# chanchanchan97/ICAFusion

Measured on AMD Instinct MI355X. Metric: RGB/IR image-pairs/sec (two-stream forward + NMS), higher is better.
Workload: dtype bf16

## Files before the change

icafusion_amd/_lib.py:

```python
import ctypes as C
import os

_HERE = os.path.dirname(os.path.abspath(__file__))
LIB_PATH = os.environ.get("ICAF_LIB") or os.path.join(_HERE, "lib", "libicaf.so")

F32, BF16, F16 = 0, 1, 2
ACT_NONE, ACT_SILU, ACT_GELU = 0, 1, 2


class ConvArgs(C.Structure):
    _fields_ = [
        ("x", C.c_void_p), ("w", C.c_void_p), ("bias", C.c_void_p), ("y", C.c_void_p), ("res", C.c_void_p),
        ("x_gs", C.c_longlong), ("w_gs", C.c_longlong), ("bias_gs", C.c_longlong), ("y_gs", C.c_longlong),
        ("res_gs", C.c_longlong),
        ("groups", C.c_int),
        ("B", C.c_int), ("H", C.c_int), ("W", C.c_int), ("Cin", C.c_int), ("ldx", C.c_int),
        ("Ho", C.c_int), ("Wo", C.c_int), ("Cout", C.c_int), ("ldy", C.c_int),
        ("kh", C.c_int), ("kw", C.c_int), ("sh", C.c_int), ("sw", C.c_int), ("ph", C.c_int), ("pw", C.c_int),
        ("ldr", C.c_int), ("Kp", C.c_int), ("act", C.c_int), ("dtype", C.c_int), ("out_dtype", C.c_int),
        ("alpha_acc", C.c_float * 2), ("alpha_res", C.c_float * 2),
        ("tile", C.c_int),
        ("pre", C.c_void_p), ("pre_h", C.c_int), ("pre_w", C.c_int), ("ldpre", C.c_int), ("pre_mode", C.c_int),
        ("w2", C.c_void_p), ("bias2", C.c_void_p), ("y2", C.c_void_p),
        ("w2_gs", C.c_longlong), ("bias2_gs", C.c_longlong), ("y2_gs", C.c_longlong),
# ... 5 lines not shown

class BneckArgs(C.Structure):
    _fields_ = [("conv", ConvArgs), ("w1", C.c_void_p), ("bias1", C.c_void_p), ("w1_gs", C.c_longlong),
                ("bias1_gs", C.c_longlong), ("Kp1", C.c_int), ("shape", C.c_int),
                ("x2", C.c_void_p), ("x2_gs", C.c_longlong), ("ldx2", C.c_int), ("reserved", C.c_int)]


class Stem2Args(C.Structure):
    _fields_ = [("img", C.c_void_p), ("img_u8", C.c_int), ("ctot", C.c_int),
                ("dtype", C.c_int), ("nstreams", C.c_int), ("B", C.c_int), ("H", C.c_int), ("W", C.c_int),
                ("w0", C.c_void_p), ("bias0", C.c_void_p), ("w0_gs", C.c_longlong), ("bias0_gs", C.c_longlong),
                ("Kp0", C.c_int), ("C0", C.c_int),
                ("w1", C.c_void_p), ("bias1", C.c_void_p), ("w1_gs", C.c_longlong), ("bias1_gs", C.c_longlong),
                ("Kp1", C.c_int), ("C1", C.c_int),
                ("w2", C.c_void_p), ("bias2", C.c_void_p), ("w2_gs", C.c_longlong), ("bias2_gs", C.c_longlong),
                ("Kp2", C.c_int), ("C2", C.c_int),
                ("y", C.c_void_p), ("y_gs", C.c_longlong), ("ldy", C.c_int), ("reserved", C.c_int)]


class DmffArgs(C.Structure):
    _fields_ = [("x", C.c_void_p), ("qkv", C.c_void_p), ("y", C.c_void_p),
                ("wqkv", C.c_void_p), ("bqkv", C.c_void_p), ("wo", C.c_void_p), ("bo", C.c_void_p),
                ("w1", C.c_void_p), ("b1", C.c_void_p), ("w2", C.c_void_p), ("b2", C.c_void_p),
                ("ln_attn_gamma", C.c_void_p * 2), ("ln_attn_beta", C.c_void_p * 2),
                ("ln_mlp_gamma", C.c_void_p), ("ln_mlp_beta", C.c_void_p),
                ("wqkv_gs", C.c_longlong), ("bqkv_gs", C.c_longlong), ("wo_gs", C.c_longlong), ("bo_gs", C.c_longlong),
                ("w1_gs", C.c_longlong), ("b1_gs", C.c_longlong), ("w2_gs", C.c_longlong), ("b2_gs", C.c_longlong),
                ("x_gs", C.c_longlong), ("y_gs", C.c_longlong),
                ("dtype", C.c_int), ("B", C.c_int), ("N", C.c_int), ("C", C.c_int), ("heads", C.c_int), ("Kp", C.c_int),
                ("Kp4", C.c_int), ("hidden", C.c_int), ("ldy", C.c_int), ("reserved", C.c_int),
                ("eps_attn", C.c_float), ("eps_mlp", C.c_float),
                ("coef_res_attn", C.c_float * 2), ("coef_acc_attn", C.c_float * 2),
                ("coef_res_mlp", C.c_float * 2), ("coef_acc_mlp", C.c_float * 2), ("debug_clock", C.c_void_p),
                ("x32", C.c_void_p), ("y32", C.c_void_p)]


class TtaPass(C.Structure):
    _fields_ = [("dst", C.c_void_p), ("Hr", C.c_int), ("Wr", C.c_int), ("Hp", C.c_int), ("Wp", C.c_int), ("flip", C.c_int), ("reserved", C.c_int)]


class FrameGeom(C.Structure):
    _fields_ = [("offset", C.c_longlong), ("h0", C.c_int), ("w0", C.c_int), ("pitch", C.c_int), ("ch", C.c_int), ("nh", C.c_int), ("nw", C.c_int),
                ("top", C.c_int), ("left", C.c_int), ("sx", C.c_float), ("sy", C.c_float)]


LETTERBOX_LDS_BYTES = 20480


_p, _i, _ll, _f, _sz = C.c_void_p, C.c_int, C.c_longlong, C.c_float, C.c_size_t
SIGNATURES = {
    "icaf_last_error": (C.c_char_p, []),
    "icaf_set_option": (_i, [C.c_char_p, _i]),
    "icaf_version": (_i, []),
    "icaf_device_info": (_i, [C.POINTER(_i), C.POINTER(_i), C.c_char_p, _i]),
    "icaf_preprocess_nchw": (_i, [_p, _p, _i, _i, _i, _i, _i, _i, _i, _p]),
    "icaf_preprocess_u8": (_i, [_p, _p, _i, _i, _i, _i, _i, _i, _i, _i, _i, _i, _p]),
    "icaf_stem": (_i, [_p, _i, _i, _p, _p, _p, _i, _i, _i, _i, _i, _i, _i, _i, _ll, _ll, _ll, _p]),
    "icaf_stem2": (_i, [C.POINTER(Stem2Args), _p]),
    "icaf_conv2d": (_i, [C.POINTER(ConvArgs), _p]),
    "icaf_bottleneck": (_i, [C.POINTER(BneckArgs), _p]),
    "icaf_conv2d_kernel_name": (_i, [C.POINTER(ConvArgs), C.c_char_p, _i]),
    "icaf_conv2d_config_ids": (_i, [C.POINTER(_i), _i]),
    "icaf_sppf_pool": (_i, [_p, _i, _p, _p, _p, _i, _i, _i, _i, _i, _i, _i, _p]),
    "icaf_sppf_config": (_i, [_i, _i, _i, _i, C.POINTER(_i)]),
    "icaf_upsample_nearest": (_i, [_p, _i, _p, _i, _i, _i, _i, _i, _i, _i, _p]),
    "icaf_copy_channels": (_i, [_p, _i, _p, _i, _i, _ll, _i, _p]),
    "icaf_axpby": (_i, [_p, _i, _p, _i, _p, _i, _i, _ll, _i, _f, _f, _p]),
    "icaf_dmff_pool_tokens": (_i, [_p, _i, _p, _i, _p, _p, _p, _i, _i, _i, _i, _i, _i, _i, _i, _i, _i, _i,
                                   _f, _f, _f, _f, _p]),
    "icaf_layernorm": (_i, [_p, _p, _p, _p, _p, _p, _i, _ll, _i, _i, _f, _p]),
    "icaf_cross_attention": (_i, [_p, _p, _i, _i, _i, _i, _i, _p]),
    "icaf_cross_attention_config": (_i, [_i, _i, _i, _i, _i, C.POINTER(_i), C.POINTER(_i), C.POINTER(_i)]),
    "icaf_dmff_ln_qkv": (_i, [C.POINTER(DmffArgs), _p]),
    "icaf_dmff_attn_mlp": (_i, [C.POINTER(DmffArgs), _p]),
    "icaf_dmff_wide_ln_qkv": (_i, [C.POINTER(DmffArgs), _p]),
    "icaf_dmff_wide_proj_mlp": (_i, [C.POINTER(DmffArgs), _p, _p]),
    "icaf_dmff_wide_proj_mlp_split": (_i, [C.POINTER(DmffArgs), _p, _p, _i, _p]),
    "icaf_dmff_wide_reduce": (_i, [C.POINTER(DmffArgs), _p, _i, _p]),
    "icaf_dmff_attn_mlp_lds_bytes": (_i, [_i, _i, _i, _i, C.POINTER(_sz)]),
    "icaf_dmff_upsample_merge": (_i, [_p, _p, _i, _p, _i, _p, _i, _i, _i, _i, _i, _i, _i, _i, _p]),
    "icaf_detect_decode": (_i, [_p, _i, _p, _p, _p, _i, _i, _i, _i, _i, _ll, _ll, _f, C.POINTER(_f), _p]),
    "icaf_detect_decode_kernel": (_i, [_p, _i, _p, _p, _i, _i, _i, _i, _i, C.POINTER(_i)]),
    "icaf_detect_conv": (_i, [C.POINTER(ConvArgs), _p, _p, _p, _i, _i, _ll, _ll, _f, C.POINTER(_f), _p]),
    "icaf_tta_stage": (_i, [_p, _i, _i, _i, _i, _i, C.POINTER(TtaPass), _i, _p]),
    "icaf_tta_merge": (_i, [C.POINTER(_p), C.POINTER(_ll), C.POINTER(_f), C.POINTER(_i), _i, _p, _i, _i, _f, _p]),
    "icaf_letterbox_frames": (_i, [_p, _p, _i, _i, _p, _i, _i, _i, _i, _p]),
    "icaf_scale_detections": (_i, [_p, _p, _i, _i, _p, _i, _p, _p]),
    "icaf_match_predictions": (_i, [_p, _p, _i, _i, _p, _p, _i, _p, _p, _i, _p, _p, _p]),
    "icaf_nms_workspace_bytes": (_i, [_i, _ll, _i, _i, C.POINTER(_sz)]),
    "icaf_nms": (_i, [_p, _i, _ll, _i, _f, _f, _i, _i, C.POINTER(_i), _i, _i, _i, _f, _p, _p, _p, _p, _sz, _p]),
    "icaf_graph_begin": (_i, [_p]),
    "icaf_graph_end": (_i, [_p, C.POINTER(_p)]),
    "icaf_graph_launch": (_i, [_p, _p]),
    "icaf_graph_destroy": (_i, [_p]),
    "icaf_event_create": (_i, [C.POINTER(_p)]),
    "icaf_event_record": (_i, [_p, _p]),
    "icaf_stream_wait_event": (_i, [_p, _p]),
    "icaf_event_elapsed_ms": (_i, [_p, _p, C.POINTER(_f)]),
    "icaf_event_destroy": (_i, [_p]),
    "icaf_stream_sync": (_i, [_p]),
}

_LIB = None


class IcafError(RuntimeError):
# ... 30 lines not shown
```

icafusion_amd/csrc/api.hip:

```cpp
#include "icaf_common.h"
#include <cstring>

namespace icaf {
std::string& last_error() {
    static thread_local std::string e;
    return e;
}
int fail(int code, const char* fmt, ...) {
    char buf[1024];
    va_list ap;
    va_start(ap, fmt);
    vsnprintf(buf, sizeof(buf), fmt, ap);
    va_end(ap);
    last_error() = buf;
    return code;
}
LibOptions g_opt;
}

using namespace icaf;

extern "C" const char* icaf_last_error(void) { return last_error().c_str(); }

extern "C" int icaf_set_option(const char* name, int value) {
    if (!name) return fail(ICAF_ERR_ARG, "icaf_set_option: null name");
    if (!strcmp(name, "detect_elementwise")) g_opt.detect_elementwise = value;
    else if (!strcmp(name, "attn_qsplit")) g_opt.attn_qsplit = value;
    else if (!strcmp(name, "sppf_vpb")) g_opt.sppf_vpb = value;
    else if (!strcmp(name, "letterbox_direct")) g_opt.letterbox_direct = value;
    else return fail(ICAF_ERR_ARG, "icaf_set_option: unknown option '%s' (detect_elementwise, attn_qsplit, sppf_vpb, letterbox_direct)", name);
    return ICAF_OK;
}
extern "C" int icaf_version(void) { return 100; }

extern "C" int icaf_device_info(int* cu_count, int* lds_bytes, char* arch, int arch_len) {
    int dev = 0;
    ICAF_HIP(hipGetDevice(&dev));
    hipDeviceProp_t prop;
    ICAF_HIP(hipGetDeviceProperties(&prop, dev));
    if (cu_count) *cu_count = prop.multiProcessorCount;
    if (lds_bytes) *lds_bytes = (int)prop.sharedMemPerBlock;
    if (arch && arch_len > 0) {
        strncpy(arch, prop.gcnArchName, arch_len - 1);
        arch[arch_len - 1] = 0;
    }
    return ICAF_OK;
}

extern "C" int icaf_graph_begin(icaf_stream_t s) {
    ICAF_HIP(hipStreamBeginCapture(S(s), hipStreamCaptureModeThreadLocal));
    return ICAF_OK;
}
extern "C" int icaf_graph_end(icaf_stream_t s, void** graph_exec) {
    hipGraph_t graph = nullptr;
    ICAF_HIP(hipStreamEndCapture(S(s), &graph));
    hipGraphExec_t exec = nullptr;
    hipError_t e = hipGraphInstantiate(&exec, graph, nullptr, nullptr, 0);
    hipGraphDestroy(graph);
    if (e != hipSuccess) return fail(ICAF_ERR_HIP, "hipGraphInstantiate -> %s", hipGetErrorString(e));
    *graph_exec = (void*)exec;
    return ICAF_OK;
}
extern "C" int icaf_graph_launch(void* graph_exec, icaf_stream_t s) {
    ICAF_HIP(hipGraphLaunch((hipGraphExec_t)graph_exec, S(s)));
    return ICAF_OK;
}
extern "C" int icaf_graph_destroy(void* graph_exec) {
    if (graph_exec) ICAF_HIP(hipGraphExecDestroy((hipGraphExec_t)graph_exec));
    return ICAF_OK;
}
extern "C" int icaf_event_create(void** ev) {
    hipEvent_t e;
    ICAF_HIP(hipEventCreate(&e));
    *ev = (void*)e;
    return ICAF_OK;
}
extern "C" int icaf_event_record(void* ev, icaf_stream_t s) {
    ICAF_HIP(hipEventRecord((hipEvent_t)ev, S(s)));
    return ICAF_OK;
}
extern "C" int icaf_stream_wait_event(icaf_stream_t s, void* ev) {
    ICAF_HIP(hipStreamWaitEvent(S(s), (hipEvent_t)ev, 0));
    return ICAF_OK;
}
extern "C" int icaf_event_elapsed_ms(void* start, void* stop, float* ms) {
    ICAF_HIP(hipEventSynchronize((hipEvent_t)stop));
// ... 12 lines not shown
```

icafusion_amd/csrc/detect.hip:

```cpp
#pragma clang fp contract(off)
#include "icaf_common.h"
#include "stream_core.h"
#include <cstdlib>

namespace icaf {

struct Anchors { float v[16]; };
int conv_prepare(const icaf_conv_args* a, ConvP& p);

struct DetectDiv { FastDiv no, nx, ny, na; };

template <bool I32>
__global__ __launch_bounds__(256) void detect_decode_kernel(const float* __restrict__ p, int ldp, float* __restrict__ z,
                                                            float* __restrict__ logits, float* __restrict__ raw, int B, int ny, int nx,
                                                            int na, int no, long long rows_total, long long row_offset, float stride,
                                                            Anchors anc, DetectDiv dv) {
    const long long total = (long long)B * na * ny * nx * no;
    for (long long e = (long long)blockIdx.x * blockDim.x + threadIdx.x; e < total; e += (long long)gridDim.x * blockDim.x) {
        int o, x, y, a, b;
        if constexpr (I32) {
            unsigned int q, r;
            fd_divmod((unsigned int)e, dv.no, q, r);
            o = (int)r;
            fd_divmod(q, dv.nx, q, r);
// ... 107 lines not shown
            const int nl = col0 + 8 * qd + 4 * hi;
#pragma unroll
            for (int b = 0; b < TM; ++b) {
                const int ml = row0 + b * 32 + l31;
                f32x4 v;
#pragma unroll
                for (int j = 0; j < 4; ++j) v[j] = acc[b][4 * qd + j] + bq[qd][j];
                *(f32x4*)(stg + ml * SO + nl * 4) = v;
            }
        }
    }
    __device__ __forceinline__ void flush(const unsigned char* stg, int m0, int n0, int tid) const {
        if (tid >= 128 * NA) return;
        const int row = tid / NA, a = tid - row * NA;
        const unsigned int pix = (unsigned int)(m0 + row);
        if ((int)pix >= M) return;
        unsigned int t, x, b, y;
        fd_divmod(pix, dnx, t, x);
        fd_divmod(t, dny, b, y);
        const float* src = (const float*)(stg + row * SO) + a * NO;
        float v[NO];
#pragma unroll
        for (int k = 0; k < NO; k += 2) { const float2 q2 = *(const float2*)(src + k); v[k] = q2.x; v[k + 1] = q2.y; }
        const long long cell = ((long long)a * ny + y) * nx + x;
        const long long zrow = (long long)b * rows_total + row_offset + cell;
        float o[NO];
#pragma unroll
        for (int k = 0; k < NO; ++k) {
            const float sg = 1.0f / (1.0f + expf(-v[k]));
            float out = sg;
            if (k == 0) out = ((sg * 2.0f - 0.5f) + (float)x) * stride;
            else if (k == 1) out = ((sg * 2.0f - 0.5f) + (float)y) * stride;
            else if (k == 2 || k == 3) {
                const float d = sg * 2.0f;
                out = (d * d) * anc.v[2 * a + (k - 2)];
            }
            o[k] = out;
        }
        float* zr = z + zrow * NO;
#pragma unroll
        for (int k = 0; k < NO; k += 2) *(float2*)(zr + k) = float2{o[k], o[k + 1]};
        if (raw) {
            float* rr = raw + (((long long)b * NA) * ny * nx + cell) * NO;
#pragma unroll
            for (int k = 0; k < NO; k += 2) *(float2*)(rr + k) = float2{v[k], v[k + 1]};
        }
        if (logits) {
#pragma unroll
            for (int k = 5; k < NO; ++k) logits[zrow * (NO - 5) + (k - 5)] = v[k];
        }
    }
};

template <int DT, int NA, int NO>
__global__ __launch_bounds__(512) void detect_conv_kernel(const ConvP p, const DetectEpi<NA, NO> epi) {
    stream_gemm<DT, 64, 1>(p, epi);
}

template <int DT, int NA, int NO>
static int launch_detect_conv(const ConvP& p, const DetectEpi<NA, NO>& epi, hipStream_t s) {
    constexpr int LDS = 3 * (128 + 64) * 128 + 128 * DetectEpi<NA, NO>::SO;
    ConvP q = p;
    q.mtiles = (p.M + 127) / 128;
    q.ntiles = 1;
    q.nchunks = p.K / 64;
    int dev = 0, cus = 256;
    ICAF_HIP(hipGetDevice(&dev));
    ICAF_HIP(hipDeviceGetAttribute(&cus, hipDeviceAttributeMultiprocessorCount, dev));
    const int grid = cus & ~7;
    ICAF_LDS_OPTIN((detect_conv_kernel<DT, NA, NO>), LDS);
    detect_conv_kernel<DT, NA, NO><<<dim3((unsigned)grid, 1, 1), dim3(512), LDS, s>>>(q, epi);
    ICAF_LAUNCH_CHECK();
    return ICAF_OK;
}

}

using namespace icaf;

enum { DETECT_PIXEL = 0, DETECT_ELEMENT = 1 };

static int detect_select(const float* p, int ldp, const float* z, const float* raw, int B, int ny, int nx, int na, int no) {
    const bool aligned = ldp % 2 == 0 && ((uintptr_t)p & 7) == 0 && ((uintptr_t)z & 7) == 0 && (!raw || ((uintptr_t)raw & 7) == 0);
    const bool pixel = na == 3 && (no == 6 || no == 8 || no == 14) && aligned && (long long)B * ny * nx < (1ll << 31) && !g_opt.detect_elementwise;
    return pixel ? DETECT_PIXEL : DETECT_ELEMENT;
}

extern "C" int icaf_detect_decode_kernel(const float* p, int ldp, const float* z, const float* raw, int B, int ny, int nx, int na, int no,
                                         int* kernel) {
    if (!p || !z || !kernel) return fail(ICAF_ERR_ARG, "icaf_detect_decode_kernel: null pointer");
    if (na < 1 || na > 8 || no < 6 || ldp < na * no) return fail(ICAF_ERR_ARG, "icaf_detect_decode_kernel: bad na/no/ldp");
    if (B < 1 || ny < 1 || nx < 1) return fail(ICAF_ERR_ARG, "icaf_detect_decode_kernel: empty level");
    *kernel = detect_select(p, ldp, z, raw, B, ny, nx, na, no);
    return ICAF_OK;
}

extern "C" int icaf_detect_decode(const float* p, int ldp, float* z, float* logits, float* raw, int B, int ny, int nx, int na, int no,
                                  long long rows_total, long long row_offset, float stride, const float* anchors_px, icaf_stream_t s) {
    if (!p || !z || !anchors_px) return fail(ICAF_ERR_ARG, "icaf_detect_decode: null pointer");
    if (na < 1 || na > 8 || no < 6 || ldp < na * no) return fail(ICAF_ERR_ARG, "icaf_detect_decode: bad na/no/ldp");
    if (row_offset + (long long)na * ny * nx > rows_total) return fail(ICAF_ERR_ARG, "icaf_detect_decode: level does not fit in z");
    Anchors anc;
    for (int i = 0; i < 16; ++i) anc.v[i] = i < 2 * na ? anchors_px[i] : 0.0f;
    const long long cells = (long long)B * na * ny * nx * no;
    long long blocks = (cells + 255) / 256;
    if (blocks > 256 * 32) blocks = 256 * 32;
    if (B < 1 || ny < 1 || nx < 1) return fail(ICAF_ERR_ARG, "icaf_detect_decode: empty level");
    if (detect_select(p, ldp, z, raw, B, ny, nx, na, no) == DETECT_PIXEL) {
        if (no == 6) return launch_detect_pixel<3, 6>(p, ldp, z, logits, raw, B, ny, nx, rows_total, row_offset, stride, anc, S(s));
        if (no == 8) return launch_detect_pixel<3, 8>(p, ldp, z, logits, raw, B, ny, nx, rows_total, row_offset, stride, anc, S(s));
        if (no == 14) return launch_detect_pixel<3, 14>(p, ldp, z, logits, raw, B, ny, nx, rows_total, row_offset, stride, anc, S(s));
    }
    const DetectDiv dv{make_fastdiv((unsigned)no), make_fastdiv((unsigned)nx), make_fastdiv((unsigned)ny), make_fastdiv((unsigned)na)};
    if (cells < (1ll << 31))
        hipLaunchKernelGGL(detect_decode_kernel<true>, dim3((unsigned)blocks), dim3(256), 0, S(s), p, ldp, z, logits, raw, B, ny, nx, na,
                           no, rows_total, row_offset, stride, anc, dv);
    else
        hipLaunchKernelGGL(detect_decode_kernel<false>, dim3((unsigned)blocks), dim3(256), 0, S(s), p, ldp, z, logits, raw, B, ny, nx, na,
                           no, rows_total, row_offset, stride, anc, dv);
    ICAF_LAUNCH_CHECK();
    return ICAF_OK;
}

extern "C" int icaf_detect_conv(const icaf_conv_args* a, float* z, float* logits, float* raw, int na, int no, long long rows_total,
                                long long row_offset, float stride, const float* anchors_px, icaf_stream_t s) {
    if (!a || !z || !anchors_px) return fail(ICAF_ERR_ARG, "icaf_detect_conv: null pointer");
// ... 25 lines not shown
```

icafusion_amd/csrc/icaf_common.h:

```cpp
#pragma once
#include <hip/hip_runtime.h>
#include <stdint.h>
#include <string>
#include <cstdio>
#include <cstdarg>
#include <atomic>
#include "../../include/icaf.h"

namespace icaf {

std::string& last_error();
int fail(int code, const char* fmt, ...);
struct LibOptions { int detect_elementwise = 0, attn_qsplit = 0, sppf_vpb = 0, letterbox_direct = 0; };
extern LibOptions g_opt;

#define ICAF_HIP(expr)                                                                        \
    do {                                                                                      \
        hipError_t _e = (expr);                                                               \
        if (_e != hipSuccess)                                                                 \
            return icaf::fail(ICAF_ERR_HIP, "%s -> %s (%s:%d)", #expr, hipGetErrorString(_e), \
                              __FILE__, __LINE__);                                            \
    } while (0)

#define ICAF_LAUNCH_CHECK() ICAF_HIP(hipGetLastError())

using u32x4 = __attribute__((ext_vector_type(4))) unsigned int;
using u32x2 = __attribute__((ext_vector_type(2))) unsigned int;
using f32x4 = __attribute__((ext_vector_type(4))) float;
using f32x16 = __attribute__((ext_vector_type(16))) float;
using bf16x8 = __attribute__((ext_vector_type(8))) __bf16;
using f16x8 = __attribute__((ext_vector_type(8))) _Float16;

__device__ __forceinline__ float bf16_to_f32(unsigned short h) { return __uint_as_float(((unsigned int)h) << 16); }
__device__ __forceinline__ unsigned short f32_to_bf16(float f) {
    return __builtin_bit_cast(unsigned short, (__bf16)f);
}
__device__ __forceinline__ unsigned int pack2_bf16(float lo, float hi) {
    using bf16x2 = __attribute__((ext_vector_type(2))) __bf16;
    bf16x2 v = {(__bf16)lo, (__bf16)hi};
    return __builtin_bit_cast(unsigned int, v);
}
__device__ __forceinline__ unsigned int pack2_f16(float lo, float hi) {
    using f16x2 = __attribute__((ext_vector_type(2))) _Float16;
    f16x2 v = {(_Float16)lo, (_Float16)hi};
    return __builtin_bit_cast(unsigned int, v);
}
__device__ __forceinline__ float f16_to_f32(unsigned short h) {
    _Float16 v = __builtin_bit_cast(_Float16, h);
    return (float)v;
}
__device__ __forceinline__ unsigned short f32_to_f16(float f) {
    _Float16 v = (_Float16)f;
    return __builtin_bit_cast(unsigned short, v);
}

template <int DT> struct Elem;
template <> struct Elem<ICAF_F32> {
    using type = float;
    static constexpr int VEC = 4;
    static constexpr int BYTES = 4;
    static __device__ __forceinline__ float ld(const float* p) { return *p; }
    static __device__ __forceinline__ void st(float* p, float v) { *p = v; }
};
template <> struct Elem<ICAF_BF16> {
    using type = unsigned short;
    static constexpr int VEC = 8;
    static constexpr int BYTES = 2;
// ... 138 lines not shown
```

icafusion_amd/csrc/igemm_stream.hip:

```cpp
#include "stream_core.h"

namespace icaf {

template <int DT, int BN, int ACT, bool PRE = false>
struct StoreEpi {
    using E = Elem<DT>;
    static constexpr int SO = BN * E::BYTES + 16;
    typename E::type* yg; float alpha_acc; int M, Cout, ldy;
    const typename E::type* rg; float alpha_res; int ldr;
    const float* pre; int pre_h, pre_w, ldpre, pre_mode, Ho, Wo;
    template <int TM>
    __device__ __forceinline__ void stage(const f32x16 (&acc)[TM], const f32x4 (&bq)[4], unsigned char* stg, int row0, int col0, int l31, int hi, int m0, int n0) const {
        const float* pt[PRE ? TM : 1][4];
        float plx[PRE ? TM : 1], ply[PRE ? TM : 1];
        if constexpr (PRE) {
#pragma clang fp contract(off)
            const float sy = (float)pre_h / (float)Ho, sx = (float)pre_w / (float)Wo;
#pragma unroll
            for (int b = 0; b < TM; ++b) {
                const int m = m0 + row0 + b * 32 + l31;
                const int mm = m < M ? m : 0;
                const int wo = mm % Wo, t = mm / Wo, ho = t % Ho, bi = t / Ho;
                float fy = ((float)ho + 0.5f) * sy - 0.5f, fx = ((float)wo + 0.5f) * sx - 0.5f;
                fy = fy < 0.0f ? 0.0f : fy;
                fx = fx < 0.0f ? 0.0f : fx;
                int y0 = (int)fy, x0 = (int)fx;
                y0 = y0 < pre_h - 1 ? y0 : pre_h - 1;
                x0 = x0 < pre_w - 1 ? x0 : pre_w - 1;
                int y1 = y0 < pre_h - 1 ? y0 + 1 : y0, x1 = x0 < pre_w - 1 ? x0 + 1 : x0;
                ply[b] = fy - (float)y0;
                plx[b] = fx - (float)x0;
                if (pre_mode == 1) {
                    y0 = y1 = (int)((long long)ho * pre_h / Ho);
                    x0 = x1 = (int)((long long)wo * pre_w / Wo);
                    ply[b] = plx[b] = 0.0f;
                }
                const float* base = pre + (long long)bi * pre_h * pre_w * ldpre;
                pt[b][0] = base + (long long)(y0 * pre_w + x0) * ldpre;
                pt[b][1] = base + (long long)(y0 * pre_w + x1) * ldpre;
                pt[b][2] = base + (long long)(y1 * pre_w + x0) * ldpre;
                pt[b][3] = base + (long long)(y1 * pre_w + x1) * ldpre;
            }
        }
#pragma unroll
        for (int qd = 0; qd < 4; ++qd) {
            const int nl = col0 + 8 * qd + 4 * hi;
#pragma unroll
            for (int b = 0; b < TM; ++b) {
                const int ml = row0 + b * 32 + l31;
                float pv[4] = {0.f, 0.f, 0.f, 0.f};
                if constexpr (PRE) if (n0 + nl < Cout) {
                    const f32x4 t00 = *(const f32x4*)(pt[b][0] + n0 + nl), t01 = *(const f32x4*)(pt[b][1] + n0 + nl);
                    const f32x4 t10 = *(const f32x4*)(pt[b][2] + n0 + nl), t11 = *(const f32x4*)(pt[b][3] + n0 + nl);
                    {
#pragma clang fp contract(off)
                        const float wx0 = 1.0f - plx[b], wy0 = 1.0f - ply[b];
#pragma unroll
                        for (int j = 0; j < 4; ++j) {
                            const float top = t00[j] * wx0 + t01[j] * plx[b];
                            const float bot = t10[j] * wx0 + t11[j] * plx[b];
                            pv[j] = top * wy0 + bot * ply[b];
                        }
                    }
                }
                float v[4];
#pragma unroll
                for (int j = 0; j < 4; ++j) v[j] = acc[b][4 * qd + j] + bq[qd][j] + pv[j];
                apply_act4<ACT, DT>(v, v);
#pragma unroll
                for (int j = 0; j < 4; ++j) v[j] *= alpha_acc;
                u32x2 pk;
                if constexpr (DT == ICAF_BF16) { pk[0] = pack2_bf16(v[0], v[1]); pk[1] = pack2_bf16(v[2], v[3]); }
                else { pk[0] = pack2_f16(v[0], v[1]); pk[1] = pack2_f16(v[2], v[3]); }
                *(u32x2*)(stg + ml * SO + nl * E::BYTES) = pk;
            }
        }
    }
    __device__ __forceinline__ void flush(const unsigned char* stg, int m0, int n0, int tid) const {
        constexpr int VPR = BN / E::VEC;
        constexpr int NIT = 128 * VPR / 512;
#pragma unroll
        for (int itv = 0; itv < NIT; ++itv) {
            const int idx = tid + itv * 512;
            const int row = idx / VPR, cv = idx - row * VPR;
            const int m = m0 + row, n = n0 + cv * E::VEC;
            u32x4 sv = *(const u32x4*)(stg + row * SO + cv * 16);
            if (m < M && n < Cout) {
                if (rg) {
                    float v[E::VEC], r[E::VEC];
                    unpack16<DT>(sv, v);
                    unpack16<DT>(*(const u32x4*)(rg + (long long)m * ldr + n), r);
#pragma unroll
                    for (int j = 0; j < E::VEC; ++j) v[j] = __builtin_fmaf(alpha_res, r[j], v[j]);
                    sv = pack16<DT>(v);
                }
                *(u32x4*)(yg + (long long)m * ldy + n) = sv;
            }
        }
    }
};

template <int DT, int BN, int ACT, int MODE, bool PRE = false>
__global__ __launch_bounds__(512) void igemm_stream_kernel(const ConvP p) {
    using E = Elem<DT>;
    const int g = blockIdx.z;
    const StoreEpi<DT, BN, ACT, PRE> epi{(typename E::type*)p.y + g * p.y_gs, p.alpha_acc[g], p.M, p.Cout, p.ldy,
                                         p.res ? (const typename E::type*)p.res + g * p.res_gs : nullptr, p.alpha_res[g], p.ldr,
                                         p.pre, p.pre_h, p.pre_w, p.ldpre, p.pre_mode, p.Ho, p.Wo};
    stream_gemm<DT, BN, MODE>(p, epi);
}

const char* stream_tag(int shape) { return shape == 1 ? "128x128" : shape == 2 ? "128x64" : "?"; }

static int stream_grid(int groups, int* wgx) {
    int dev = 0, cus = 256;
    ICAF_HIP(hipGetDevice(&dev));
    ICAF_HIP(hipDeviceGetAttribute(&cus, hipDeviceAttributeMultiprocessorCount, dev));
    *wgx = ((cus / (groups > 0 ? groups : 1)) & ~7) >> 3;
    return ICAF_OK;
}

int stream_check(const icaf_conv_args* a, const ConvP& p, int shape) {
    if (shape < 1 || shape > 2) return fail(ICAF_ERR_ARG, "igemm_stream: unknown shape %d", shape);
    if (a->dtype == ICAF_F32 || a->out_dtype != a->dtype) return fail(ICAF_ERR_UNSUPPORTED, "igemm_stream: 16-bit types, out dtype == dtype");
    if ((a->Cin * 2) % 128) return fail(ICAF_ERR_UNSUPPORTED, "igemm_stream: Cin * 2 bytes must be a multiple of 128 (Cin = %d)", a->Cin);
    if (a->w2) return fail(ICAF_ERR_UNSUPPORTED, "igemm_stream: no chained layer");
    if (a->pre && (a->act != ICAF_ACT_SILU || a->kh != 1 || a->kw != 1 || a->sh != 1 || a->sw != 1 || a->ph || a->pw || a->groups != 1))
        return fail(ICAF_ERR_UNSUPPORTED, "igemm_stream: the pre-activation term is built for 1x1 SiLU layers (one group)");
    if (a->res && !p.vec_r) return fail(ICAF_ERR_UNSUPPORTED, "igemm_stream: the residual must take 16-byte vectors");
    if (p.x_bytes == 0) return fail(ICAF_ERR_UNSUPPORTED, "igemm_stream: operand exceeds the 2 GiB buffer-descriptor range");
    if (!p.vec_y || a->Cout % 8) return fail(ICAF_ERR_UNSUPPORTED, "igemm_stream: y must take 16-byte vectors (ldy %% 8, Cout %% 8, alignment)");
    if (shape == 1 && a->Cout <= 64) return fail(ICAF_ERR_UNSUPPORTED, "igemm_stream 128x128: Cout = %d <= 64 (use 128x64)", a->Cout);
    int wgx = 0;
    const int st = stream_grid(a->groups, &wgx);
    if (st) return st;
    const int ntiles = (p.Cout + (shape == 1 ? 128 : 64) - 1) / (shape == 1 ? 128 : 64);
    if (wgx < ntiles || wgx % ntiles) return fail(ICAF_ERR_UNSUPPORTED, "igemm_stream: %d channel tiles do not divide the %d workgroups of an XCD", ntiles, wgx);
    return ICAF_OK;
}

template <int DT, int BN, int ACT>
static int launch_stream_cfg(const ConvP& p, int groups, hipStream_t s) {
    constexpr int LDS = 3 * (128 + BN) * 128 + 128 * (BN * 2 + 16);
    ConvP q = p;
    q.mtiles = (p.M + 127) / 128;
    q.ntiles = (p.Cout + BN - 1) / BN;
    q.nchunks = p.K / 64;
    int dev = 0, wgx = 0;
    ICAF_HIP(hipGetDevice(&dev));
    if (dev < 0 || dev >= ICAF_MAX_DEVICES) return fail(ICAF_ERR_UNSUPPORTED, "device ordinal %d", dev);
    int st = stream_grid(groups, &wgx);
    if (st) return st;
    const int grid = wgx << 3;
    if (wgx < q.ntiles || wgx % q.ntiles) return fail(ICAF_ERR_UNSUPPORTED, "igemm_stream: %d channel tiles do not divide the %d workgroups of an XCD", q.ntiles, wgx);
    const bool plain = q.kh == 1 && q.kw == 1 && q.sh == 1 && q.sw == 1 && q.ph == 0 && q.pw == 0;
    auto go = [&](auto kern) -> int {
        ICAF_LDS_OPTIN(kern, LDS);
        kern<<<dim3((unsigned)grid, 1, (unsigned)groups), dim3(512), LDS, s>>>(q);
        ICAF_LAUNCH_CHECK();
        return ICAF_OK;
    };
    if constexpr (ACT == ICAF_ACT_SILU) { if (p.pre) return go(igemm_stream_kernel<DT, BN, ACT, 1, true>); }
    if (plain) return go(igemm_stream_kernel<DT, BN, ACT, 1>);
    return go(igemm_stream_kernel<DT, BN, ACT, 2>);
}

template <int DT, int BN>
static int launch_stream_act(const ConvP& p, int groups, hipStream_t s) {
    if (p.act == ICAF_ACT_SILU) return launch_stream_cfg<DT, BN, ICAF_ACT_SILU>(p, groups, s);
    if (p.act == ICAF_ACT_GELU) return launch_stream_cfg<DT, BN, ICAF_ACT_GELU>(p, groups, s);
    return launch_stream_cfg<DT, BN, ICAF_ACT_NONE>(p, groups, s);
}

int launch_stream(const icaf_conv_args* a, const ConvP& p, int shape, hipStream_t s) {
    if (a->dtype == ICAF_BF16) return shape == 1 ? launch_stream_act<ICAF_BF16, 128>(p, a->groups, s) : launch_stream_act<ICAF_BF16, 64>(p, a->groups, s);
    return shape == 1 ? launch_stream_act<ICAF_F16, 128>(p, a->groups, s) : launch_stream_act<ICAF_F16, 64>(p, a->groups, s);
}

}
```

icafusion_amd/csrc/stream_core.h:

```cpp
#pragma once
#include "conv_common.h"

namespace icaf {

template <int DT, int BN, int MODE, class EPI>
__device__ __forceinline__ void stream_gemm(const ConvP& p, const EPI& epi) {
    using E = Elem<DT>;
    static_assert(DT != ICAF_F32, "16-bit types");
    constexpr int BM = 128, RB = 128, NS = 3, NW = 8;
    constexpr int WN = 32, WM = BN == 128 ? 64 : 32;
    constexpr int TM = WM / 32, TN = 1;
    constexpr int WAVES_M = BM / WM;
    constexpr int VEC = E::VEC;
    constexpr int RPI = 8;
    constexpr int NA = BM / RPI / NW, NB = BN / RPI / NW;
    constexpr int PER = NA + NB;
    constexpr int STAGE = (BM + BN) * RB;
    constexpr int NSTEP = RB / 32;
    constexpr int RING = NS * STAGE;
    static_assert(NA >= 1 && NB >= 1 && (BN == 128 || BN == 64), "tile shape");
    extern __shared__ __attribute__((aligned(1024))) unsigned char lds[];
    unsigned char* stg = lds + RING;

    const int tid = threadIdx.x, lane = tid & 63, l31 = lane & 31, hi = lane >> 5;
    const int wave = __builtin_amdgcn_readfirstlane(tid >> 6);
    const int g = blockIdx.z;
    const int wm = wave % WAVES_M, wn = wave / WAVES_M;

    const __amdgpu_buffer_rsrc_t xr = __builtin_amdgcn_make_buffer_rsrc(
        (void*)((const typename E::type*)p.x + g * p.x_gs), 0, p.x_bytes, 0x00020000);
    const __amdgpu_buffer_rsrc_t wr = __builtin_amdgcn_make_buffer_rsrc(
        (void*)((const typename E::type*)p.w + g * p.w_gs), 0, p.w_bytes, 0x00020000);
    constexpr unsigned OOB = 0x80000000u;

    const int rsub = lane >> 3;
    const int dkey = ((wave & 1) << 2) | (rsub >> 1);
    const int lslot = (lane & 7) ^ dkey;

    const int xcd = blockIdx.x & 7, lb = blockIdx.x >> 3, wgx = gridDim.x >> 3;
    const int per_xcd = (p.mtiles + 7) >> 3, m_lo = xcd * per_xcd, m_hi = min(m_lo + per_xcd, p.mtiles);
    const int nt = lb % p.ntiles, mstride = wgx / p.ntiles, m_first = m_lo + lb / p.ntiles;
    const int n0 = nt * BN;
    const int nch = p.nchunks;

    int it = m_first, ic = 0;
    int kc = 0, ky = 0, kx = 0;
    unsigned ia_off[NA], iw_off[NB];
    int ia_h0[NA], ia_w0[NA];
#pragma unroll
    for (int i = 0; i < NB; ++i)
        iw_off[i] = ((unsigned)(n0 + (wave + NW * i) * RPI + rsub) * (unsigned)p.Kp + (unsigned)(lslot * VEC)) * E::BYTES;
    auto issue_setup = [&]() {
        const bool live = it < m_hi;
#pragma unroll
        for (int i = 0; i < NA; ++i) {
            const int m = it * BM + (wave + NW * i) * RPI + rsub;
            const bool ok = live && m < p.M;
            if constexpr (MODE == 1) {
                ia_off[i] = ok ? ((unsigned)m * (unsigned)p.ldx + (unsigned)(lslot * VEC)) * E::BYTES : OOB;
            } else {
                const int mm = ok ? m : 0;
                const int wo = mm % p.Wo, t = mm / p.Wo, ho = t % p.Ho, b = t / p.Ho;
                ia_h0[i] = ok ? ho * p.sh - p.ph : -0x10000;
                ia_w0[i] = wo * p.sw - p.pw;
                ia_off[i] = (unsigned)b * (unsigned)(p.H * p.W) * (unsigned)p.ldx * (unsigned)E::BYTES
                          + (unsigned)((ia_h0[i] * p.W + ia_w0[i]) * p.ldx + lslot * VEC) * E::BYTES;
            }
        }
    };
    auto issue_part = [&](int stage, int part) {
        unsigned char* st = lds + stage * STAGE;
        const unsigned koff = (unsigned)ic * RB;
        unsigned tap_delta = 0;
        if constexpr (MODE == 2) tap_delta = (unsigned)((ky * p.W + kx) * p.ldx + kc) * E::BYTES;
#pragma unroll
        for (int i = 0; i < NA; ++i) {
            if (i % NSTEP != part) continue;
            unsigned voff;
            if constexpr (MODE == 1) {
                voff = ia_off[i] == OOB ? OOB : ia_off[i] + koff;
            } else {
                const int h = ia_h0[i] + ky, w = ia_w0[i] + kx;
                const bool ok = (unsigned)h < (unsigned)p.H && (unsigned)w < (unsigned)p.W;
                voff = ok ? ia_off[i] + tap_delta : OOB;
            }
            __builtin_amdgcn_raw_ptr_buffer_load_lds(xr, (lds_ptr_t)(st + (wave + NW * i) * 1024), 16, voff, 0, 0, 0);
        }
#pragma unroll
        for (int i = 0; i < NB; ++i) {
            if ((NA + i) % NSTEP != part) continue;
            const unsigned voff = it < m_hi ? iw_off[i] + koff : OOB;
            __builtin_amdgcn_raw_ptr_buffer_load_lds(wr, (lds_ptr_t)(st + BM * RB + (wave + NW * i) * 1024), 16, voff, 0, 0, 0);
        }
    };
    auto issue_advance = [&]() {
        if constexpr (MODE == 2) {
            kc += RB / E::BYTES;
            if (kc >= p.Cin) { kc = 0; if (++kx == p.kw) { kx = 0; ++ky; } }
        }
        if (++ic == nch) {
            ic = 0; kc = 0; ky = 0; kx = 0;
            it += mstride;
            issue_setup();
        }
    };

    const float* __restrict__ bias = p.bias ? p.bias + g * p.bias_gs : nullptr;
    f32x4 bq[4];
#pragma unroll
    for (int qd = 0; qd < 4; ++qd) {
        const int n = n0 + wn * WN + 8 * qd + 4 * hi;
        const bool okn = bias && n < p.Cout;
        const float* bp = okn ? bias + n : (const float*)p.w;
        const f32x4 t = *(const f32x4*)bp;
        bq[qd] = okn ? t : f32x4{0.f, 0.f, 0.f, 0.f};
    }
#pragma unroll
    for (int qd = 0; qd < 4; ++qd) asm volatile("" : "+v"(bq[qd]));

    if (m_first >= m_hi) return;

    const int fkey = (l31 >> 1) & 7;
    int foff[NSTEP];
#pragma unroll
    for (int s = 0; s < NSTEP; ++s) foff[s] = l31 * RB + (((2 * s + hi) ^ fkey) << 4);

    issue_setup();
#pragma unroll
    for (int s = 0; s < NS; ++s) {
#pragma unroll
        for (int part = 0; part < NSTEP; ++part) issue_part(s, part);
        issue_advance();
    }

    int q = 0;
    for (int mt = m_first; mt < m_hi; mt += mstride) {
        const int m0 = mt * BM;
        f32x16 acc[TM];
#pragma unroll
        for (int b = 0; b < TM; ++b)
#pragma unroll
            for (int r = 0; r < 16; ++r) acc[b][r] = 0.0f;
        for (int c = 0; c < nch; ++c, ++q) {
            wait_vmcnt<PER>();
            asm volatile("s_waitcnt lgkmcnt(0)" ::: "memory");
            __builtin_amdgcn_s_barrier();
            const int sq = q % NS;
            const unsigned char* a_s = lds + sq * STAGE;
            const unsigned char* b_s = a_s + BM * RB;
            u32x4 fp[NSTEP][TM], fw[NSTEP];
#pragma unroll
            for (int s = 0; s < NSTEP; ++s) {
#pragma unroll
                for (int b = 0; b < TM; ++b) fp[s][b] = *(const u32x4*)(a_s + (wm * WM + b * 32) * RB + foff[s]);
                fw[s] = *(const u32x4*)(b_s + (wn * WN) * RB + foff[s]);
            }
            const int sfree = (q + NS - 1) % NS;
#pragma unroll
            for (int s = 0; s < NSTEP; ++s) {
#pragma unroll
                for (int b = 0; b < TM; ++b) mma_step<DT>(acc[b], fw[s], fp[s][b]);
                if (q > 0) issue_part(sfree, s);
            }
            if (q > 0) issue_advance();
        }

        epi.stage(acc, bq, stg, wm * WM, wn * WN, l31, hi, m0, n0);
        lds_barrier();
        epi.flush(stg, m0, n0, tid);
    }
    wait_vmcnt<0>();
}


}
```

icafusion_amd/ops.py:

```python
import collections
import contextlib
import ctypes as C
import weakref

import numpy as np
import torch

from . import _lib
from .options import OPT
from ._lib import BneckArgs, ConvArgs, DmffArgs, FrameGeom, Stem2Args, check, lib, F32, BF16, F16, ACT_NONE, ACT_SILU, ACT_GELU

_DT = {torch.float32: F32, torch.bfloat16: BF16, torch.float16: F16}
VEC = {torch.float32: 4, torch.bfloat16: 8, torch.float16: 8}
N_ALIGN = 128
K_ALIGN_BYTES = 128


def dtype_code(dt):
    try:
        return _DT[dt]
    except KeyError:
        raise _lib.IcafError(f"unsupported dtype {dt}; supported: float32, bfloat16, float16") from None


# ... 823 lines not shown

def geom_tensor(geom, device=None, pin=False):
    t = torch.from_numpy(np.ascontiguousarray(geom).view(np.uint8).reshape(-1).copy())
    if device is not None:
        return t.to(device)
    return t.pin_memory() if pin else t


def letterbox_frames(arena, geom, geom_dev, dst, swap_rb=True, c0=0, name="letterbox_frames"):
    if arena.dtype != torch.uint8 or not arena.is_contiguous() or arena.dim() != 1:
        raise ValueError("the arena must be a flat contiguous uint8 tensor")
    if dst.dtype != torch.uint8 or not dst.is_contiguous() or dst.dim() != 4:
        raise ValueError("dst must be a contiguous uint8 (B, ctot, H, W) tensor")
    B, ctot, H, W = dst.shape
    n = len(geom)
    if n % B or n == 0 or 3 * (n // B) > ctot:
        raise ValueError(f"{n} descriptors for a batch of {B} images with {ctot} channels")
    if W % 16:
        raise ValueError(f"output width {W} must be a multiple of 16")
    if geom_dev.numel() * geom_dev.element_size() < n * GEOM_DTYPE.itemsize:
        raise ValueError("the device table is smaller than the descriptor rows")
    validate_frames(geom, arena.numel(), H, W)
    if not (arena.is_cuda and dst.is_cuda and geom_dev.is_cuda):
        raise ValueError("arena, table and dst must be cuda tensors (no CPU fallback exists)")
    nb = sum(int(g["h0"]) * int(g["w0"]) * int(g["ch"]) for g in geom) + n * 3 * H * W
    return Launch(lib().icaf_letterbox_frames, (arena.data_ptr(), geom_dev.data_ptr(), n // B, B, dst.data_ptr(), ctot, H, W, int(bool(swap_rb))),
                  keep=(arena, geom_dev, dst), name=name, nbytes=nb)


def scale_detections(det, count, scale, out=None, round=False, name="scale_detections"):
    out = det if out is None else out
    if det.dim() != 3 or det.shape[2] != 6 or det.dtype != torch.float32 or not det.is_contiguous() or not det.is_cuda:
        raise ValueError("det must be a contiguous cuda float32 (B, max_det, 6) tensor")
    if out.shape != det.shape or out.dtype != det.dtype or not out.is_contiguous() or out.device != det.device:
        raise ValueError("out must match det")
    B, max_det, _ = det.shape
    if count.dtype != torch.int32 or count.numel() != B or not count.is_contiguous() or count.device != det.device:
        raise ValueError("count must be a cuda int32 (B,) tensor")
    if scale.dtype != torch.float32 or tuple(scale.shape) != (B, 5) or not scale.is_contiguous() or scale.device != det.device:
        raise ValueError("scale must be a cuda float32 (B, 5) tensor of {gain, pad_x, pad_y, w0, h0} rows")
    return Launch(lib().icaf_scale_detections, (det.data_ptr(), count.data_ptr(), B, max_det, scale.data_ptr(), int(bool(round)), out.data_ptr()),
                  keep=(det, count, scale, out), name=name, nbytes=2 * det.numel() * 4)


@contextlib.contextmanager
def letterbox_direct(on=True):
    check(lib().icaf_set_option(b"letterbox_direct", int(bool(on))), "icaf_set_option(letterbox_direct)")
    try:
        yield
    finally:
        check(lib().icaf_set_option(b"letterbox_direct", 0), "icaf_set_option(letterbox_direct)")


def match_predictions(det, count, labels, label_off, iouv, scale=None, predn=None, stream_ptr=None):
    B, max_det, six = det.shape
    assert six == 6 and det.dtype == torch.float32 and det.is_contiguous() and count.dtype == torch.int32
    assert label_off.dtype == torch.int32 and label_off.numel() == B + 1 and iouv.dtype == torch.float32
    assert labels.dtype == torch.float32 and labels.is_contiguous() and (labels.numel() == 0 or labels.shape[1] == 5)
    T = iouv.numel()
    correct = torch.empty((B, max_det, T), dtype=torch.uint8, device=det.device)
    off = label_off.cpu()
    max_l = int((off[1:] - off[:-1]).max()) if B else 0
    st = lib().icaf_match_predictions(det.data_ptr(), count.data_ptr(), B, max_det, labels.data_ptr() if labels.numel() else None,
                                      label_off.data_ptr(), max_l, scale.data_ptr() if scale is not None else None, iouv.data_ptr(), T,
                                      correct.data_ptr(), predn.data_ptr() if predn is not None else None,
                                      stream_ptr if stream_ptr is not None else current_stream_ptr())
    check(st, "icaf_match_predictions")
    return correct


class Graph:
    def __init__(self):
        self.exec = C.c_void_p(None)

    def capture(self, stream_ptr, fn):
        check(lib().icaf_graph_begin(stream_ptr), "graph_begin")
        try:
            fn()
        finally:
            st = lib().icaf_graph_end(stream_ptr, C.byref(self.exec))
        check(st, "graph_end")

    def launch(self, stream_ptr):
        check(lib().icaf_graph_launch(self.exec, stream_ptr), "graph_launch")

    def __del__(self):
        try:
            if self.exec:
                lib().icaf_graph_destroy(self.exec)
        except Exception:
            pass


class Event:
    def __init__(self):
        self.ev = C.c_void_p(None)
        check(lib().icaf_event_create(C.byref(self.ev)), "event_create")

    def record(self, stream_ptr):
        check(lib().icaf_event_record(self.ev, stream_ptr), "event_record")

    def wait(self, stream_ptr):
        check(lib().icaf_stream_wait_event(stream_ptr, self.ev), "stream_wait_event")

    def elapsed_ms(self, stop):
        ms = C.c_float(0)
# ... 16 lines not shown
```

include/icaf.h:

```cpp
#ifndef ICAF_H
#define ICAF_H

#include <stddef.h>

#ifdef __cplusplus
extern "C" {
#endif

typedef void* icaf_stream_t;

enum { ICAF_F32 = 0, ICAF_BF16 = 1, ICAF_F16 = 2 };
enum { ICAF_ACT_NONE = 0, ICAF_ACT_SILU = 1, ICAF_ACT_GELU = 2 };
enum { ICAF_OK = 0, ICAF_ERR_ARG = -1, ICAF_ERR_HIP = -2, ICAF_ERR_UNSUPPORTED = -3 };

const char* icaf_last_error(void);
int icaf_set_option(const char* name, int value);
int icaf_version(void);
int icaf_device_info(int* cu_count, int* lds_bytes, char* arch, int arch_len);

int icaf_preprocess_nchw(const float* img, void* out, int dtype, int B, int C, int H, int W, int Cpad, int mode,
                         icaf_stream_t s);
int icaf_preprocess_u8(const unsigned char* img, void* out, int dtype, int B, int Ctot, int c0, int C, int nstreams,
                       int H, int W, int Cpad, int mode, icaf_stream_t s);

int icaf_stem(const void* img, int img_u8, int ctot, const void* w, const float* bias, void* y, int ldy, int dtype,
              int nstreams, int B, int H, int W, int Cout, int Kp, long long w_gs, long long bias_gs, long long y_gs,
              icaf_stream_t s);

typedef struct icaf_stem2_args {
    const void* img; int img_u8, ctot;
    int dtype, nstreams, B, H, W;
    const void* w0; const float* bias0; long long w0_gs, bias0_gs; int Kp0, C0;
    const void* w1; const float* bias1; long long w1_gs, bias1_gs; int Kp1, C1;
    const void* w2; const float* bias2; long long w2_gs, bias2_gs; int Kp2, C2;
    void* y; long long y_gs; int ldy, reserved;
} icaf_stem2_args;
int icaf_stem2(const icaf_stem2_args* a, icaf_stream_t s);

typedef struct icaf_conv_args {
    const void* x;
    const void* w;
    const float* bias;
    void* y;
    const void* res;
    long long x_gs, w_gs, bias_gs, y_gs, res_gs;
    int groups;
    int B, H, W, Cin, ldx;
    int Ho, Wo, Cout, ldy;
    int kh, kw, sh, sw, ph, pw;
    int ldr;
    int Kp;
    int act;
    int dtype;
    int out_dtype;
    float alpha_acc[2];
    float alpha_res[2];
    int tile;
    const float* pre;
    int pre_h, pre_w, ldpre;
    int pre_mode;
    const void* w2;
    const float* bias2;
    void* y2;
    long long w2_gs, bias2_gs, y2_gs;
    int Kp2, Cout2, ldy2;
    int chain_keep;
    const void* wf;
    long long wf_gs;
    const void* x2;
    long long x2_gs;
// ... 125 lines not shown
```

Baseline: 16610.

## Keep whole weight panel resident in LDS for plain 1x1 stream GEMMs

Adds a resident form of the persistent stream GEMM. When the full BN x K weight panel fits within a 160 KB LDS budget, it is loaded into LDS once per workgroup and the pipeline ring stages carry only activation tiles. This removes the per-k-step weight reloads and shrinks each stage, at the cost of more LDS per workgroup, which may lower occupancy, plus a longer prologue. It is enabled by default for plain 1x1 convolutions and the detect head, and can be switched off through a new runtime option.

Result: no change. 16700, median of 6 (+0.5%).

```diff
diff --git a/icafusion_amd/_lib.py b/icafusion_amd/_lib.py
--- a/icafusion_amd/_lib.py
+++ b/icafusion_amd/_lib.py
@@ -81,6 +81,7 @@
     "icaf_last_error": (C.c_char_p, []),
     "icaf_set_option": (_i, [C.c_char_p, _i]),
     "icaf_version": (_i, []),
+    "icaf_stream_config": (_i, [_i, _i, _i, C.POINTER(_i), C.POINTER(_i)]),
     "icaf_device_info": (_i, [C.POINTER(_i), C.POINTER(_i), C.c_char_p, _i]),
     "icaf_preprocess_nchw": (_i, [_p, _p, _i, _i, _i, _i, _i, _i, _i, _p]),
     "icaf_preprocess_u8": (_i, [_p, _p, _i, _i, _i, _i, _i, _i, _i, _i, _i, _i, _p]),
diff --git a/icafusion_amd/csrc/api.hip b/icafusion_amd/csrc/api.hip
--- a/icafusion_amd/csrc/api.hip
+++ b/icafusion_amd/csrc/api.hip
@@ -28,10 +28,21 @@
     else if (!strcmp(name, "attn_qsplit")) g_opt.attn_qsplit = value;
     else if (!strcmp(name, "sppf_vpb")) g_opt.sppf_vpb = value;
     else if (!strcmp(name, "letterbox_direct")) g_opt.letterbox_direct = value;
-    else return fail(ICAF_ERR_ARG, "icaf_set_option: unknown option '%s' (detect_elementwise, attn_qsplit, sppf_vpb, letterbox_direct)", name);
+    else if (!strcmp(name, "stream_resident")) g_opt.stream_resident = value;
+    else return fail(ICAF_ERR_ARG, "icaf_set_option: unknown option '%s' (detect_elementwise, attn_qsplit, sppf_vpb, letterbox_direct, stream_resident)", name);
     return ICAF_OK;
 }
 extern "C" int icaf_version(void) { return 100; }
+
+extern "C" int icaf_stream_config(int bn, int K, int staging_bytes, int* stages, int* lds_bytes) {
+    if (!stages || !lds_bytes) return fail(ICAF_ERR_ARG, "icaf_stream_config: null pointer");
+    if ((bn != 64 && bn != 128) || K < 64 || K % 64 || K > (1 << 20) || staging_bytes < 0 || staging_bytes > STREAM_LDS_BUDGET)
+        return fail(ICAF_ERR_ARG, "icaf_stream_config: bn in {64, 128}, K a multiple of 64, 0 <= staging <= %d (bn = %d, K = %d, staging = %d)",
+                    STREAM_LDS_BUDGET, bn, K, staging_bytes);
+    *stages = stream_stages(bn, K, staging_bytes);
+    *lds_bytes = *stages ? stream_lds_bytes(bn, K, staging_bytes, *stages) : 3 * (128 + bn) * 128 + staging_bytes;
+    return ICAF_OK;
+}
 
 extern "C" int icaf_device_info(int* cu_count, int* lds_bytes, char* arch, int arch_len) {
     int dev = 0;
diff --git a/icafusion_amd/csrc/detect.hip b/icafusion_amd/csrc/detect.hip
--- a/icafusion_amd/csrc/detect.hip
+++ b/icafusion_amd/csrc/detect.hip
@@ -183,14 +183,15 @@
     }
 };
 
-template <int DT, int NA, int NO>
+template <int DT, int NA, int NO, bool RES = false>
 __global__ __launch_bounds__(512) void detect_conv_kernel(const ConvP p, const DetectEpi<NA, NO> epi) {
-    stream_gemm<DT, 64, 1>(p, epi);
+    stream_gemm<DT, 64, 1, DetectEpi<NA, NO>, RES>(p, epi);
 }
 
 template <int DT, int NA, int NO>
 static int launch_detect_conv(const ConvP& p, const DetectEpi<NA, NO>& epi, hipStream_t s) {
-    constexpr int LDS = 3 * (128 + 64) * 128 + 128 * DetectEpi<NA, NO>::SO;
+    constexpr int STG = 128 * DetectEpi<NA, NO>::SO;
+    constexpr int LDS = 3 * (128 + 64) * 128 + STG;
     ConvP q = p;
     q.mtiles = (p.M + 127) / 128;
     q.ntiles = 1;
@@ -199,10 +200,15 @@
     ICAF_HIP(hipGetDevice(&dev));
     ICAF_HIP(hipDeviceGetAttribute(&cus, hipDeviceAttributeMultiprocessorCount, dev));
     const int grid = cus & ~7;
-    ICAF_LDS_OPTIN((detect_conv_kernel<DT, NA, NO>), LDS);
-    detect_conv_kernel<DT, NA, NO><<<dim3((unsigned)grid, 1, 1), dim3(512), LDS, s>>>(q, epi);
-    ICAF_LAUNCH_CHECK();
-    return ICAF_OK;
+    auto go = [&](auto kern, int lds) -> int {
+        ICAF_LDS_OPTIN(kern, lds);
+        kern<<<dim3((unsigned)grid, 1, 1), dim3(512), lds, s>>>(q, epi);
+        ICAF_LAUNCH_CHECK();
+        return ICAF_OK;
+    };
+    const int ns = g_opt.stream_resident ? stream_stages(64, p.K, STG) : 0;
+    if (ns) return go(detect_conv_kernel<DT, NA, NO, true>, stream_lds_bytes(64, p.K, STG, ns));
+    return go(detect_conv_kernel<DT, NA, NO>, LDS);
 }
 
 }
diff --git a/icafusion_amd/csrc/icaf_common.h b/icafusion_amd/csrc/icaf_common.h
--- a/icafusion_amd/csrc/icaf_common.h
+++ b/icafusion_amd/csrc/icaf_common.h
@@ -11,8 +11,14 @@
 
 std::string& last_error();
 int fail(int code, const char* fmt, ...);
-struct LibOptions { int detect_elementwise = 0, attn_qsplit = 0, sppf_vpb = 0, letterbox_direct = 0; };
+struct LibOptions { int detect_elementwise = 0, attn_qsplit = 0, sppf_vpb = 0, letterbox_direct = 0, stream_resident = 1; };
 extern LibOptions g_opt;
+
+constexpr int STREAM_LDS_BUDGET = 160 * 1024, STREAM_STAGE_BYTES = 128 * 128, STREAM_STAGES = 3;
+constexpr int stream_stages(int bn, int K, int staging) {
+    return (long long)STREAM_STAGES * STREAM_STAGE_BYTES + (long long)bn * K * 2 + staging <= STREAM_LDS_BUDGET ? STREAM_STAGES : 0;
+}
+constexpr int stream_lds_bytes(int bn, int K, int staging, int stages) { return stages * STREAM_STAGE_BYTES + staging + bn * K * 2; }
 
 #define ICAF_HIP(expr)                                                                        \
     do {                                                                                      \
diff --git a/icafusion_amd/csrc/igemm_stream.hip b/icafusion_amd/csrc/igemm_stream.hip
--- a/icafusion_amd/csrc/igemm_stream.hip
+++ b/icafusion_amd/csrc/igemm_stream.hip
@@ -6,6 +6,8 @@
 struct StoreEpi {
     using E = Elem<DT>;
     static constexpr int SO = BN * E::BYTES + 16;
+    static_assert(stream_stages(128, 256, 128 * 272) == 3 && stream_stages(128, 320, 128 * 272) == 0 && stream_stages(64, 704, 128 * 144) == 3 &&
+                  stream_stages(64, 768, 128 * 144) == 0, "where the resident form ends for this epilogue");
     typename E::type* yg; float alpha_acc; int M, Cout, ldy;
     const typename E::type* rg; float alpha_res; int ldr;
     const float* pre; int pre_h, pre_w, ldpre, pre_mode, Ho, Wo;
@@ -100,14 +102,14 @@
     }
 };
 
-template <int DT, int BN, int ACT, int MODE, bool PRE = false>
+template <int DT, int BN, int ACT, int MODE, bool PRE = false, bool RES = false>
 __global__ __launch_bounds__(512) void igemm_stream_kernel(const ConvP p) {
     using E = Elem<DT>;
     const int g = blockIdx.z;
     const StoreEpi<DT, BN, ACT, PRE> epi{(typename E::type*)p.y + g * p.y_gs, p.alpha_acc[g], p.M, p.Cout, p.ldy,
                                          p.res ? (const typename E::type*)p.res + g * p.res_gs : nullptr, p.alpha_res[g], p.ldr,
                                          p.pre, p.pre_h, p.pre_w, p.ldpre, p.pre_mode, p.Ho, p.Wo};
-    stream_gemm<DT, BN, MODE>(p, epi);
+    stream_gemm<DT, BN, MODE, StoreEpi<DT, BN, ACT, PRE>, RES>(p, epi);
 }
 
 const char* stream_tag(int shape) { return shape == 1 ? "128x128" : shape == 2 ? "128x64" : "?"; }
@@ -141,7 +143,8 @@
 
 template <int DT, int BN, int ACT>
 static int launch_stream_cfg(const ConvP& p, int groups, hipStream_t s) {
-    constexpr int LDS = 3 * (128 + BN) * 128 + 128 * (BN * 2 + 16);
+    constexpr int STG = 128 * (BN * 2 + 16);
+    constexpr int LDS = 3 * (128 + BN) * 128 + STG;
     ConvP q = p;
     q.mtiles = (p.M + 127) / 128;
     q.ntiles = (p.Cout + BN - 1) / BN;
@@ -154,15 +157,19 @@
     const int grid = wgx << 3;
     if (wgx < q.ntiles || wgx % q.ntiles) return fail(ICAF_ERR_UNSUPPORTED, "igemm_stream: %d channel tiles do not divide the %d workgroups of an XCD", q.ntiles, wgx);
     const bool plain = q.kh == 1 && q.kw == 1 && q.sh == 1 && q.sw == 1 && q.ph == 0 && q.pw == 0;
-    auto go = [&](auto kern) -> int {
-        ICAF_LDS_OPTIN(kern, LDS);
-        kern<<<dim3((unsigned)grid, 1, (unsigned)groups), dim3(512), LDS, s>>>(q);
+    auto go = [&](auto kern, int lds) -> int {
+        ICAF_LDS_OPTIN(kern, lds);
+        kern<<<dim3((unsigned)grid, 1, (unsigned)groups), dim3(512), lds, s>>>(q);
         ICAF_LAUNCH_CHECK();
         return ICAF_OK;
     };
-    if constexpr (ACT == ICAF_ACT_SILU) { if (p.pre) return go(igemm_stream_kernel<DT, BN, ACT, 1, true>); }
-    if (plain) return go(igemm_stream_kernel<DT, BN, ACT, 1>);
-    return go(igemm_stream_kernel<DT, BN, ACT, 2>);
+    if constexpr (ACT == ICAF_ACT_SILU) { if (p.pre) return go(igemm_stream_kernel<DT, BN, ACT, 1, true>, LDS); }
+    if (plain) {
+        const int ns = g_opt.stream_resident ? stream_stages(BN, p.K, STG) : 0;
+        if (ns) return go(igemm_stream_kernel<DT, BN, ACT, 1, false, true>, stream_lds_bytes(BN, p.K, STG, ns));
+        return go(igemm_stream_kernel<DT, BN, ACT, 1>, LDS);
+    }
+    return go(igemm_stream_kernel<DT, BN, ACT, 2>, LDS);
 }
 
 template <int DT, int BN>
diff --git a/icafusion_amd/csrc/stream_core.h b/icafusion_amd/csrc/stream_core.h
--- a/icafusion_amd/csrc/stream_core.h
+++ b/icafusion_amd/csrc/stream_core.h
@@ -3,24 +3,28 @@
 
 namespace icaf {
 
-template <int DT, int BN, int MODE, class EPI>
+template <int DT, int BN, int MODE, class EPI, bool RES = false>
 __device__ __forceinline__ void stream_gemm(const ConvP& p, const EPI& epi) {
     using E = Elem<DT>;
     static_assert(DT != ICAF_F32, "16-bit types");
+    static_assert(!RES || MODE == 1, "the resident form is built for plain 1x1 launches");
     constexpr int BM = 128, RB = 128, NS = 3, NW = 8;
     constexpr int WN = 32, WM = BN == 128 ? 64 : 32;
     constexpr int TM = WM / 32, TN = 1;
     constexpr int WAVES_M = BM / WM;
     constexpr int VEC = E::VEC;
     constexpr int RPI = 8;
-    constexpr int NA = BM / RPI / NW, NB = BN / RPI / NW;
+    constexpr int NA = BM / RPI / NW, NWT = BN / RPI / NW;
+    constexpr int NB = RES ? 0 : NWT;
     constexpr int PER = NA + NB;
-    constexpr int STAGE = (BM + BN) * RB;
+    constexpr int STAGE = (BM + (RES ? 0 : BN)) * RB;
     constexpr int NSTEP = RB / 32;
     constexpr int RING = NS * STAGE;
-    static_assert(NA >= 1 && NB >= 1 && (BN == 128 || BN == 64), "tile shape");
+    static_assert(NA >= 1 && NWT >= 1 && (BN == 128 || BN == 64), "tile shape");
     extern __shared__ __attribute__((aligned(1024))) unsigned char lds[];
     unsigned char* stg = lds + RING;
+    unsigned char* wts = stg + BM * EPI::SO;
+    static_assert((BM * EPI::SO) % 1024 == 0, "the weight region starts on a DMA instruction's 1 KB");
 
     const int tid = threadIdx.x, lane = tid & 63, l31 = lane & 31, hi = lane >> 5;
     const int wave = __builtin_amdgcn_readfirstlane(tid >> 6);
@@ -45,10 +49,10 @@
 
     int it = m_first, ic = 0;
     int kc = 0, ky = 0, kx = 0;
-    unsigned ia_off[NA], iw_off[NB];
+    unsigned ia_off[NA], iw_off[NWT];
     int ia_h0[NA], ia_w0[NA];
 #pragma unroll
-    for (int i = 0; i < NB; ++i)
+    for (int i = 0; i < NWT; ++i)
         iw_off[i] = ((unsigned)(n0 + (wave + NW * i) * RPI + rsub) * (unsigned)p.Kp + (unsigned)(lslot * VEC)) * E::BYTES;
     auto issue_setup = [&]() {
         const bool live = it < m_hi;
@@ -125,6 +129,14 @@
 #pragma unroll
     for (int s = 0; s < NSTEP; ++s) foff[s] = l31 * RB + (((2 * s + hi) ^ fkey) << 4);
 
+    if constexpr (RES) {
+        for (int c = 0; c < nch; ++c)
+#pragma unroll
+            for (int i = 0; i < NWT; ++i)
+                __builtin_amdgcn_raw_ptr_buffer_load_lds(wr, (lds_ptr_t)(wts + c * (BN * RB) + (wave + NW * i) * 1024), 16,
+                                                         iw_off[i] + (unsigned)c * RB, 0, 0, 0);
+    }
+
     issue_setup();
 #pragma unroll
     for (int s = 0; s < NS; ++s) {
@@ -133,6 +145,7 @@
         issue_advance();
     }
 
+    if constexpr (RES) wait_vmcnt<NS * NA>();
     int q = 0;
     for (int mt = m_first; mt < m_hi; mt += mstride) {
         const int m0 = mt * BM;
@@ -147,7 +160,7 @@
             __builtin_amdgcn_s_barrier();
             const int sq = q % NS;
             const unsigned char* a_s = lds + sq * STAGE;
-            const unsigned char* b_s = a_s + BM * RB;
+            const unsigned char* b_s = RES ? wts + c * (BN * RB) : a_s + BM * RB;
             u32x4 fp[NSTEP][TM], fw[NSTEP];
 #pragma unroll
             for (int s = 0; s < NSTEP; ++s) {
diff --git a/icafusion_amd/ops.py b/icafusion_amd/ops.py
--- a/icafusion_amd/ops.py
+++ b/icafusion_amd/ops.py
@@ -899,6 +899,24 @@
         check(lib().icaf_set_option(b"letterbox_direct", 0), "icaf_set_option(letterbox_direct)")
 
 
+@contextlib.contextmanager
+def stream_resident(on=True):
+    check(lib().icaf_set_option(b"stream_resident", int(bool(on))), "icaf_set_option(stream_resident)")
+    try:
+        yield
+    finally:
+        check(lib().icaf_set_option(b"stream_resident", 1), "icaf_set_option(stream_resident)")
+
+
+STREAM_LDS_BUDGET = 160 * 1024
+
+
+def stream_config(bn, K, staging_bytes):
+    st, nb = C.c_int(0), C.c_int(0)
+    check(lib().icaf_stream_config(int(bn), int(K), int(staging_bytes), C.byref(st), C.byref(nb)), "icaf_stream_config")
+    return st.value, nb.value
+
+
 def match_predictions(det, count, labels, label_off, iouv, scale=None, predn=None, stream_ptr=None):
     B, max_det, six = det.shape
     assert six == 6 and det.dtype == torch.float32 and det.is_contiguous() and count.dtype == torch.int32
diff --git a/include/icaf.h b/include/icaf.h
--- a/include/icaf.h
+++ b/include/icaf.h
@@ -16,6 +16,7 @@
 const char* icaf_last_error(void);
 int icaf_set_option(const char* name, int value);
 int icaf_version(void);
+int icaf_stream_config(int bn, int K, int staging_bytes, int* stages, int* lds_bytes);
 int icaf_device_info(int* cu_count, int* lds_bytes, char* arch, int arch_len);
 
 int icaf_preprocess_nchw(const float* img, void* out, int dtype, int B, int C, int H, int W, int Cpad, int mode,
```
